# GLAD-RUC/DistEGNN

Hardware: NVIDIA H100
Metric: graph_steps_per_sec (higher is better)
Workload: dtype f32

## Files before the change

### distegnn_b200/csrc/edge_layer_cs.cu

```cuda
#include <cuda_fp16.h>
#include <string.h>

#include "common.cuh"
#include "det.cuh"
#include "tc16.cuh"
#include "tile_mma.cuh"

namespace degnn {

struct EdgeCsArgs {
    int64_t N, E;
    const int32_t* E_dev;
    int A;
    unsigned flags;
    const int32_t* row;
    const int32_t* col;
    const float* ea;
    const float* x4;
    const float* P;
    const float* Q;
    const float* w1r;
    const float* w1e;
    const float* w2;
    const float* b2;
    const float* wc;
    const float* bc;
    const float* w3;
    float* agg_m;
    float* agg_x;
    float* slots;
};

constexpr int CS_WG = 4;
constexpr int CS_THREADS = 128 * CS_WG, CS_WARPS = CS_THREADS / 32;
constexpr int CS_TILE = 64;
constexpr int CS_QROW = 72;
constexpr int CS_WBUF = 16 * CS_QROW;
constexpr int CS_IDX = 64;
constexpr int CS_W = 64 * 64;
constexpr int CS_SMEM_BYTES = 4 * CS_W * 2
                              + CS_WARPS * 2 * 8
                              + (4 * H + DISTEGNN_MAX_EDGE_ATTR * H) * 4
                              + CS_WARPS * 2 * CS_WBUF * 4
                              + CS_WARPS * CS_IDX * 4
                              + CS_WARPS * 16 * 8 * 4;
constexpr uint32_t CS_LBO = 1024;

template <int AT, bool LASTL, bool DET>
__global__ void __launch_bounds__(CS_THREADS, 1) edge_layer_cs_kernel(const EdgeCsArgs a) {
    using namespace tmma;
    constexpr int AMAX = AT >= 0 ? (AT > 0 ? AT : 1) : DISTEGNN_MAX_EDGE_ATTR;
    constexpr int AR = (AT == 1 || AT == 2) ? AT : 0;
    constexpr bool need_m = !LASTL;
    __half* W2hi = reinterpret_cast<__half*>(degnn_dyn_smem);
    __half* W2lo = W2hi + CS_W;
    __half* Wchi = W2lo + CS_W;
    __half* Wclo = Wchi + CS_W;
    uint64_t* bars = reinterpret_cast<uint64_t*>(Wclo + CS_W);
    float* b2s = reinterpret_cast<float*>(bars + CS_WARPS * 2);
    float* bcs = b2s + H;
    float* w3s = bcs + H;
    float* w1rs = w3s + H;
    float* w1es = w1rs + H;
    float* qbufs = w1es + DISTEGNN_MAX_EDGE_ATTR * H;
    int* idx_all = reinterpret_cast<int*>(qbufs + CS_WARPS * 2 * CS_WBUF);
    float* xs_all = reinterpret_cast<float*>(idx_all + CS_WARPS * CS_IDX);

    const int tid = threadIdx.x;
    const int lane = tid & 31;
    const int warp = tid >> 5;
    const int wg = warp >> 2;
    const int w = warp & 3;
    const int g = lane >> 2, q = lane & 3;
    const int A = AT >= 0 ? AT : a.A;
    const bool normalize = a.flags & DISTEGNN_FLAG_NORMALIZE;

    tc16::stage_weight<CS_THREADS>(W2hi, W2lo, a.w2, 0, 64, tid, SILU_T_IN);
    tc16::stage_weight<CS_THREADS>(Wchi, Wclo, a.wc, 0, 64, tid);
    if (tid < H) {
        b2s[tid] = a.b2[tid] * SILU_T_IN;
        bcs[tid] = a.bc[tid] * SILU_T_IN;
        w3s[tid] = a.w3[tid] * SILU_T_OUT;
        w1rs[tid] = a.w1r[tid];
    }
    for (int i = tid; i < DISTEGNN_MAX_EDGE_ATTR * H; i += CS_THREADS) w1es[i] = i < A * H ? a.w1e[i] : 0.f;
    for (int i = tid; i < CS_WARPS * 2 * CS_WBUF / 4; i += CS_THREADS)
        reinterpret_cast<float4*>(qbufs)[i] = make_float4(0.f, 0.f, 0.f, 0.f);
    if (tid == 0) {
        for (int i = 0; i < CS_WARPS * 2; ++i) mbar_init(&bars[i], 1);
        fence_mbar_init();
    }
    fence_proxy_async_smem();
    __syncthreads();

    float* qb = qbufs + warp * 2 * CS_WBUF;
    int* nidx = idx_all + warp * CS_IDX;
    float* xs = xs_all + warp * 16 * 8 + 8 * (lane & 15);
    uint64_t* qbar = bars + 2 * warp;
    const uint64_t bW2hi = make_desc(smem_u32(W2hi), CS_LBO, 128), bW2lo = make_desc(smem_u32(W2lo), CS_LBO, 128);
    const uint64_t bWchi = make_desc(smem_u32(Wchi), CS_LBO, 128), bWclo = make_desc(smem_u32(Wclo), CS_LBO, 128);

    const int64_t nE = a.E_dev ? min((int64_t)__ldg(a.E_dev), a.E) : a.E;
    const int64_t num_tiles = (nE + CS_TILE - 1) / CS_TILE;
    const int64_t stride = (int64_t)gridDim.x * CS_WG;
    int64_t tile = (int64_t)blockIdx.x * CS_WG + wg;

    auto edge_of = [&](int64_t tl) { return tl * CS_TILE + 16 * w + lane; };
    auto has_edge = [&](int64_t tl) { return lane < 16 && tl < num_tiles && edge_of(tl) < nE; };
    auto fetch_q = [&](int64_t tl, int b, int col_e, bool v) {
        if (lane == 0) {
            const int64_t nv = min((int64_t)16, max((int64_t)0, nE - (tl * CS_TILE + 16 * w)));
            mbar_expect_tx(qbar + b, (uint32_t)nv * (H * 4));
        }
        if (v) bulk_g2s(qb + b * CS_WBUF + lane * CS_QROW, a.Q + (size_t)col_e * H, H * 4, qbar + b);
    };

    int row_c = -1;
    float dx = 0.f, dy = 0.f, dz = 0.f, radial = 0.f;
    auto set_geometry = [&](float4 xi, float4 xj) {
        dx = xi.x - xj.x; dy = xi.y - xj.y; dz = xi.z - xj.z;
        radial = dx * dx + dy * dy + dz * dz;
        if (normalize) {
            const float inv = 1.0f / (sqrtf(radial) + 1e-8f);
            dx *= inv; dy *= inv; dz *= inv;
        }
    };
    float ea_c[AR > 0 ? AR : 1], n_ea[AR > 0 ? AR : 1];
#pragma unroll
    for (int k = 0; k < (AR > 0 ? AR : 1); ++k) ea_c[k] = n_ea[k] = 0.f;
    int n_row = -1, n_col = 0;

    if (tile < num_tiles) {
        int col_c = 0;
        if (has_edge(tile)) {
            const int64_t e = edge_of(tile);
            row_c = __ldg(a.row + e);
            col_c = __ldg(a.col + e);
#pragma unroll
            for (int k = 0; k < AR; ++k) ea_c[k] = __ldg(a.ea + e * AR + k);
        }
        fetch_q(tile, 0, col_c, row_c >= 0);
        set_geometry(ldg4(a.x4 + (size_t)max(row_c, 0) * 4), ldg4(a.x4 + (size_t)col_c * 4));
        if (has_edge(tile + stride)) {
            const int64_t e = edge_of(tile + stride);
            n_row = __ldg(a.row + e);
            n_col = __ldg(a.col + e);
#pragma unroll
            for (int k = 0; k < AR; ++k) n_ea[k] = __ldg(a.ea + e * AR + k);
        }
    }

    for (int it = 0; tile < num_tiles; ++it, tile += stride) {
        const int64_t ntile = tile + stride, nntile = ntile + stride;
        const int b = it & 1;
        float* qcur = qb + b * CS_WBUF;

        int cont_row = -1;
        if constexpr (DET) {
            const int64_t e0 = tile * CS_TILE + 16 * w;
            const int r0 = __shfl_sync(FULL, row_c, 0);
            if (r0 >= 0 && e0 > 0 && __ldg(a.row + e0 - 1) == r0) cont_row = r0;
        }
        float* const slot = DET ? a.slots + (size_t)(tile * 4 + w) * DET_EDGE_SLOT : nullptr;

        if (ntile < num_tiles) fetch_q(ntile, b ^ 1, n_col, n_row >= 0);
        if (n_row >= 0) {
            cp_async16(xs, a.x4 + (size_t)n_row * 4);
            cp_async16(xs + 4, a.x4 + (size_t)n_col * 4);
            prefetch_l1(a.P + (size_t)n_row * H);
            prefetch_l1(a.P + (size_t)n_row * H + 32);
        }
        if (has_edge(nntile)) {
            const int64_t e = edge_of(nntile);
            cp_async4(nidx + lane, a.row + e);
            cp_async4(nidx + 16 + lane, a.col + e);
            if (AT == 1) cp_async4(nidx + 32 + 2 * lane, a.ea + e);
            if (AT == 2) cp_async8(nidx + 32 + 2 * lane, a.ea + e * 2);
        }
        cp_async_commit();

        const int ra = __shfl_sync(FULL, row_c, g), rb = __shfl_sync(FULL, row_c, g + 8);
        const float rada = __shfl_sync(FULL, radial, g), radb = __shfl_sync(FULL, radial, g + 8);
        float eaa[AMAX], eab[AMAX];
#pragma unroll
        for (int k = 0; k < AMAX; ++k) {
            if (AR > 0) {
                eaa[k] = __shfl_sync(FULL, ea_c[k < AR ? k : 0], g);
                eab[k] = __shfl_sync(FULL, ea_c[k < AR ? k : 0], g + 8);
            } else if (AT < 0) {
                const int64_t e = tile * CS_TILE + 16 * w + g;
                eaa[k] = (k < A && ra >= 0) ? __ldg(a.ea + e * A + k) : 0.f;
                eab[k] = (k < A && rb >= 0) ? __ldg(a.ea + (e + 8) * A + k) : 0.f;
            } else {
                eaa[k] = eab[k] = 0.f;
            }
        }
        const float* pa = a.P + (size_t)max(ra, 0) * H + 2 * q;
        const float* pb = a.P + (size_t)max(rb, 0) * H + 2 * q;
        const float* qa = qcur + g * CS_QROW + 2 * q;
        const float* qbr = qa + 8 * CS_QROW;
        const bool oka = !DET || ra >= 0, okb = !DET || rb >= 0;
        auto pre = [&](int j, const float* prow, const float* qrow, float rad, const float (&ea)[AMAX], bool ok) {
            if (DET && !ok) return bc2(0.f);
            const int c = 8 * j + 2 * q;
            const f32x2 pp = __ldg(reinterpret_cast<const f32x2*>(prow + 8 * j));
            const f32x2 qq = *reinterpret_cast<const f32x2*>(qrow + 8 * j);
            f32x2 p = fma2(bc2(rad), *reinterpret_cast<const f32x2*>(w1rs + c), add2(pp, qq));
#pragma unroll
            for (int k = 0; k < AMAX; ++k)
                if (AT < 0 || k < A)
                    p = fma2(bc2(ea[k]), *reinterpret_cast<const f32x2*>(w1es + k * H + c), p);
            return p;
        };
        uint32_t ahi[16], alo[16];
        float qmax = 0.f;
        auto silu_guard = [&] { return silu_q_overflow(qmax); };
        tc16::RowScales s1;
        mbar_wait(qbar + b, (uint32_t)((it >> 1) & 1));
        tc16::encode_rows<false, true>(
            [&](int j, f32x2& va, f32x2& vb, auto pass) {
                va = pre(j, pa, qa, rada, eaa, oka);
                vb = pre(j, pb, qbr, radb, eab, okb);
                silu4p<decltype(pass)::value != tc16::FAST_PASS>(va, vb, qmax);
            },
            ahi, alo, s1, silu_guard);

        float d[32];
        tc16::mma_f16x3_rA<CS_LBO>(d, ahi, alo, bW2hi, bW2lo);
        const int row_prev = __shfl_up_sync(FULL, row_c, 1);
        const uint32_t M = __ballot_sync(FULL, lane == 0 || row_prev != row_c) & 0xffffu;
        tc16::mma_f16x3_rA_wait(d, ahi, alo);

        qmax = 0.f;
        tc16::RowScales s2;
        tc16::encode_rows<false>(
            [&](int j, f32x2& ma, f32x2& mb, auto pass) {
                const f32x2 bb = *reinterpret_cast<const f32x2*>(b2s + 8 * j + 2 * q);
                ma = fma2(pk2(d[4 * j + 0], d[4 * j + 1]), bc2(s1.inv_a), bb);
                mb = fma2(pk2(d[4 * j + 2], d[4 * j + 3]), bc2(s1.inv_b), bb);
                silu4t<decltype(pass)::value != tc16::FAST_PASS>(ma, mb, qmax);
                if (need_m && decltype(pass)::value != tc16::ENCODE_PASS) {
                    *reinterpret_cast<f32x2*>(qcur + g * CS_QROW + 8 * j + 2 * q) = ma;
                    *reinterpret_cast<f32x2*>(qcur + (g + 8) * CS_QROW + 8 * j + 2 * q) = mb;
                }
            },
            ahi, alo, s2, silu_guard);

        tc16::mma_f16x3_rA<CS_LBO>(d, ahi, alo, bWchi, bWclo);
        if (need_m) {
            __syncwarp();
            const float* colp = qcur + 2 * lane;
            auto flush = [&](f32x2 acc, int e_last) {
                const int rr = __shfl_sync(FULL, row_c, e_last);
                if (rr >= 0) {
                    float v0, v1;
                    upk2(mul2(acc, bc2(SILU_T_OUT)), v0, v1);
                    if constexpr (DET)
                        *reinterpret_cast<float2*>(rr == cont_row ? slot + 2 * lane : a.agg_m + (size_t)rr * H + 2 * lane) =
                            make_float2(v0, v1);
                    else
                        red_add_v2(a.agg_m + (size_t)rr * H + 2 * lane, v0, v1);
                }
            };
            f32x2 s0 = *reinterpret_cast<const f32x2*>(colp);
            if ((M >> 1) == 0u) {
                f32x2 s1 = *reinterpret_cast<const f32x2*>(colp + CS_QROW);
#pragma unroll
                for (int e = 2; e < 16; e += 2) {
                    s0 = add2(s0, *reinterpret_cast<const f32x2*>(colp + e * CS_QROW));
                    s1 = add2(s1, *reinterpret_cast<const f32x2*>(colp + (e + 1) * CS_QROW));
                }
                flush(add2(s0, s1), 15);
            } else {
#pragma unroll
                for (int e = 1; e < 16; ++e) {
                    const f32x2 v = *reinterpret_cast<const f32x2*>(colp + e * CS_QROW);
                    if ((M >> e) & 1u) {
                        flush(s0, e - 1);
                        s0 = v;
                    } else {
                        s0 = add2(s0, v);
                    }
                }
                flush(s0, 15);
            }
        }
        fence_proxy_async_smem();
        __syncwarp();
        tc16::mma_f16x3_rA_wait(d, ahi, alo);

        float phia, phib;
        tc16::phi_head_t(d, s2.inv_a, s2.inv_b, bcs, w3s, q, phia, phib);
        {
            const float fa = __shfl_sync(FULL, phia, 4 * (lane & 7)), fb = __shfl_sync(FULL, phib, 4 * (lane & 7));
            const float phi = (lane & 8) ? fb : fa;
            float sx = dx * phi, sy = dy * phi, sz = dz * phi;
#pragma unroll
            for (int o = 1; o < 16; o <<= 1) {
                const int rk = __shfl_up_sync(FULL, row_c, o);
                const float ox = __shfl_up_sync(FULL, sx, o), oy = __shfl_up_sync(FULL, sy, o), oz = __shfl_up_sync(FULL, sz, o);
                if (lane >= o && rk == row_c) { sx += ox; sy += oy; sz += oz; }
            }
            const int rnext = __shfl_down_sync(FULL, row_c, 1);
            if (row_c >= 0 && (lane == 15 || rnext != row_c)) {
                if constexpr (DET) {
                    float* dst = row_c == cont_row ? slot + H : a.agg_x + (size_t)row_c * 4;
                    dst[0] = sx;
                    dst[1] = sy;
                    dst[2] = sz;
                } else {
                    float* dst = a.agg_x + (size_t)row_c * 4;
                    atomicAdd(dst + 0, sx);
                    atomicAdd(dst + 1, sy);
                    atomicAdd(dst + 2, sz);
                }
            }
        }

        cp_async_wait_all();
        row_c = n_row;
        float4 xi_n = make_float4(0.f, 0.f, 0.f, 0.f), xj_n = xi_n;
        if (n_row >= 0) {
            xi_n = *reinterpret_cast<const float4*>(xs);
            xj_n = *reinterpret_cast<const float4*>(xs + 4);
        }
        set_geometry(xi_n, xj_n);
#pragma unroll
        for (int k = 0; k < AR; ++k) ea_c[k] = n_ea[k];
        n_row = -1;
        if (has_edge(nntile)) {
            n_row = nidx[lane];
            n_col = nidx[16 + lane];
            if (AT == 1) n_ea[0] = __int_as_float(nidx[32 + 2 * lane]);
            if (AT == 2) {
                n_ea[0] = __int_as_float(nidx[32 + 2 * lane]);
                n_ea[AR - 1] = __int_as_float(nidx[33 + 2 * lane]);
            }
        }
    }
}

}

namespace degnn {

template <bool DET>
static int edge_layer_fwd(int64_t n_nodes, int64_t n_edges, int A, int C, int Na, unsigned flags, const int32_t* row,
                          const int32_t* col, const float* edge_attr_sorted, const float* x4, const float* P,
                          const float* Q, const float* layer_params, float* agg_m, float* agg_x,
                          const int32_t* n_edges_dev, void* workspace, int64_t workspace_bytes, void* stream,
                          int max_ctas) {
    if (int rc = check_dims(A, C, Na)) return rc;
    if (n_edges == 0) return DISTEGNN_OK;
    DEGNN_CHECK_ARG(n_nodes > 0 && n_edges > 0, "negative size");
    DEGNN_CHECK_ARG(row && col && x4 && P && Q && layer_params && agg_x, "null pointer");
    DEGNN_CHECK_ARG(A == 0 || edge_attr_sorted, "null edge_attr with edge_attr_nf > 0");
    DEGNN_CHECK_ARG((flags & DISTEGNN_FLAG_LAST) || agg_m, "null agg_m");
    float* slots = nullptr;
    if (DET) {
        if (int rc = det_check_workspace(n_nodes, n_edges, C, workspace, workspace_bytes, "distegnn_edge_layer_fwd_det"))
            return rc;
        slots = det_edge_slots(workspace, n_nodes, C);
    }
    Layout L = make_layout(A, C, Na);
    EdgeCsArgs a;
    a.N = n_nodes; a.E = n_edges; a.E_dev = n_edges_dev; a.A = A; a.flags = flags & 0xffffu;
    a.row = row; a.col = col; a.ea = edge_attr_sorted; a.x4 = x4; a.P = P; a.Q = Q;
    a.w1r = layer_params + L.off[DISTEGNN_P_E_W1R];
    a.w1e = layer_params + L.off[DISTEGNN_P_E_W1E];
    a.w2 = layer_params + L.off[DISTEGNN_P_E_W2];
    a.b2 = layer_params + L.off[DISTEGNN_P_E_B2];
    a.wc = layer_params + L.off[DISTEGNN_P_E_WC];
    a.bc = layer_params + L.off[DISTEGNN_P_E_BC];
    a.w3 = layer_params + L.off[DISTEGNN_P_E_W3];
    a.agg_m = agg_m; a.agg_x = agg_x; a.slots = slots;
    const int64_t tiles = (n_edges + CS_TILE - 1) / CS_TILE;
    int64_t grid = (tiles + CS_WG - 1) / CS_WG;
    if (grid > sm_count()) grid = sm_count();
    if (DET) grid = det_grid(grid, max_ctas);
    auto launch = [&](auto kern) {
        ensure_dynamic_smem((const void*)kern, (int)CS_SMEM_BYTES);
        kern<<<(unsigned)grid, CS_THREADS, CS_SMEM_BYTES, (cudaStream_t)stream>>>(a);
    };
    const bool last = flags & DISTEGNN_FLAG_LAST;
    switch (A) {
        case 0: last ? launch(edge_layer_cs_kernel<0, true, DET>) : launch(edge_layer_cs_kernel<0, false, DET>); break;
        case 1: last ? launch(edge_layer_cs_kernel<1, true, DET>) : launch(edge_layer_cs_kernel<1, false, DET>); break;
        case 2: last ? launch(edge_layer_cs_kernel<2, true, DET>) : launch(edge_layer_cs_kernel<2, false, DET>); break;
        default: last ? launch(edge_layer_cs_kernel<-1, true, DET>) : launch(edge_layer_cs_kernel<-1, false, DET>); break;
    }
    DEGNN_CHECK_LAUNCH();
    return DISTEGNN_OK;
}

int edge_layer_fwd_det(int64_t n_nodes, int64_t n_edges, int A, int C, int Na, unsigned flags, const int32_t* row,
                       const int32_t* col, const float* edge_attr_sorted, const float* x4, const float* P, const float* Q,
                       const float* layer_params, float* agg_m, float* agg_x, const int32_t* n_edges_dev,
                       void* workspace, int64_t workspace_bytes, void* stream, int max_ctas) {
    return edge_layer_fwd<true>(n_nodes, n_edges, A, C, Na, flags, row, col, edge_attr_sorted, x4, P, Q, layer_params,
                                agg_m, agg_x, n_edges_dev, workspace, workspace_bytes, stream, max_ctas);
}

}

extern "C" int distegnn_edge_layer_fwd(int64_t n_nodes, int64_t n_edges, int A, int C, int Na, unsigned flags,
                                       const int32_t* row, const int32_t* col, const float* edge_attr_sorted,
                                       const float* x4, const float* P, const float* Q,
                                       const float* layer_params, float* agg_m, float* agg_x,
                                       const int32_t* n_edges_dev, void* stream) {
    return degnn::edge_layer_fwd<false>(n_nodes, n_edges, A, C, Na, flags, row, col, edge_attr_sorted, x4, P, Q,
                                        layer_params, agg_m, agg_x, n_edges_dev, nullptr, 0, stream, 0);
}

extern "C" int distegnn_edge_layer_fwd_det(int64_t n_nodes, int64_t n_edges, int A, int C, int Na, unsigned flags,
                                           const int32_t* row, const int32_t* col, const float* edge_attr_sorted,
                                           const float* x4, const float* P, const float* Q,
                                           const float* layer_params, float* agg_m, float* agg_x,
                                           const int32_t* n_edges_dev, void* workspace, int64_t workspace_bytes,
                                           void* stream) {
    return degnn::edge_layer_fwd_det(n_nodes, n_edges, A, C, Na, flags, row, col, edge_attr_sorted, x4, P, Q,
                                     layer_params, agg_m, agg_x, n_edges_dev, workspace, workspace_bytes, stream, 0);
}
```

Before: 34.55.

## Replace TMA bulk Q-row fetch with warp-cooperative cp.async and defer issue

Drops the per-warp mbarriers and TMA bulk_g2s copies of gathered Q rows. Each warp now fetches the rows with 16-byte cp.async, lanes cooperating two rows per step via shuffles, and completion is tracked through the existing cp.async group wait. For fixed attribute counts, issuing the next tile's prefetches is moved to after the first MMA is launched, so they overlap tensor-core work. This removes mbarrier wait and proxy-fence overhead but adds more per-lane instructions and shuffles, and the Q data must now arrive within the same tile iteration.

```diff
diff --git a/distegnn_b200/csrc/edge_layer_cs.cu b/distegnn_b200/csrc/edge_layer_cs.cu
--- a/distegnn_b200/csrc/edge_layer_cs.cu
+++ b/distegnn_b200/csrc/edge_layer_cs.cu
@@ -39,7 +39,6 @@
 constexpr int CS_IDX = 64;
 constexpr int CS_W = 64 * 64;
 constexpr int CS_SMEM_BYTES = 4 * CS_W * 2
-                              + CS_WARPS * 2 * 8
                               + (4 * H + DISTEGNN_MAX_EDGE_ATTR * H) * 4
                               + CS_WARPS * 2 * CS_WBUF * 4
                               + CS_WARPS * CS_IDX * 4
@@ -56,8 +55,7 @@
     __half* W2lo = W2hi + CS_W;
     __half* Wchi = W2lo + CS_W;
     __half* Wclo = Wchi + CS_W;
-    uint64_t* bars = reinterpret_cast<uint64_t*>(Wclo + CS_W);
-    float* b2s = reinterpret_cast<float*>(bars + CS_WARPS * 2);
+    float* b2s = reinterpret_cast<float*>(Wclo + CS_W);
     float* bcs = b2s + H;
     float* w3s = bcs + H;
     float* w1rs = w3s + H;
@@ -86,17 +84,12 @@
     for (int i = tid; i < DISTEGNN_MAX_EDGE_ATTR * H; i += CS_THREADS) w1es[i] = i < A * H ? a.w1e[i] : 0.f;
     for (int i = tid; i < CS_WARPS * 2 * CS_WBUF / 4; i += CS_THREADS)
         reinterpret_cast<float4*>(qbufs)[i] = make_float4(0.f, 0.f, 0.f, 0.f);
-    if (tid == 0) {
-        for (int i = 0; i < CS_WARPS * 2; ++i) mbar_init(&bars[i], 1);
-        fence_mbar_init();
-    }
     fence_proxy_async_smem();
     __syncthreads();
 
     float* qb = qbufs + warp * 2 * CS_WBUF;
     int* nidx = idx_all + warp * CS_IDX;
     float* xs = xs_all + warp * 16 * 8 + 8 * (lane & 15);
-    uint64_t* qbar = bars + 2 * warp;
     const uint64_t bW2hi = make_desc(smem_u32(W2hi), CS_LBO, 128), bW2lo = make_desc(smem_u32(W2lo), CS_LBO, 128);
     const uint64_t bWchi = make_desc(smem_u32(Wchi), CS_LBO, 128), bWclo = make_desc(smem_u32(Wclo), CS_LBO, 128);
 
@@ -107,12 +100,12 @@
 
     auto edge_of = [&](int64_t tl) { return tl * CS_TILE + 16 * w + lane; };
     auto has_edge = [&](int64_t tl) { return lane < 16 && tl < num_tiles && edge_of(tl) < nE; };
-    auto fetch_q = [&](int64_t tl, int b, int col_e, bool v) {
-        if (lane == 0) {
-            const int64_t nv = min((int64_t)16, max((int64_t)0, nE - (tl * CS_TILE + 16 * w)));
-            mbar_expect_tx(qbar + b, (uint32_t)nv * (H * 4));
-        }
-        if (v) bulk_g2s(qb + b * CS_WBUF + lane * CS_QROW, a.Q + (size_t)col_e * H, H * 4, qbar + b);
+    auto fetch_q = [&](int b, int col_v) {
+#pragma unroll
+        for (int i = 0; i < 8; ++i) {
+            const int r = 2 * i + (lane >> 4), c = __shfl_sync(FULL, col_v, r);
+            if (c >= 0) cp_async16(qb + b * CS_WBUF + r * CS_QROW + 4 * (lane & 15), a.Q + (size_t)c * H + 4 * (lane & 15));
+        }
     };
 
     int row_c = -1;
@@ -139,7 +132,8 @@
 #pragma unroll
             for (int k = 0; k < AR; ++k) ea_c[k] = __ldg(a.ea + e * AR + k);
         }
-        fetch_q(tile, 0, col_c, row_c >= 0);
+        fetch_q(0, row_c >= 0 ? col_c : -1);
+        cp_async_commit();
         set_geometry(ldg4(a.x4 + (size_t)max(row_c, 0) * 4), ldg4(a.x4 + (size_t)col_c * 4));
         if (has_edge(tile + stride)) {
             const int64_t e = edge_of(tile + stride);
@@ -148,6 +142,8 @@
 #pragma unroll
             for (int k = 0; k < AR; ++k) n_ea[k] = __ldg(a.ea + e * AR + k);
         }
+        cp_async_wait_all();
+        __syncwarp();
     }
 
     for (int it = 0; tile < num_tiles; ++it, tile += stride) {
@@ -163,21 +159,24 @@
         }
         float* const slot = DET ? a.slots + (size_t)(tile * 4 + w) * DET_EDGE_SLOT : nullptr;
 
-        if (ntile < num_tiles) fetch_q(ntile, b ^ 1, n_col, n_row >= 0);
-        if (n_row >= 0) {
-            cp_async16(xs, a.x4 + (size_t)n_row * 4);
-            cp_async16(xs + 4, a.x4 + (size_t)n_col * 4);
-            prefetch_l1(a.P + (size_t)n_row * H);
-            prefetch_l1(a.P + (size_t)n_row * H + 32);
-        }
-        if (has_edge(nntile)) {
-            const int64_t e = edge_of(nntile);
-            cp_async4(nidx + lane, a.row + e);
-            cp_async4(nidx + 16 + lane, a.col + e);
-            if (AT == 1) cp_async4(nidx + 32 + 2 * lane, a.ea + e);
-            if (AT == 2) cp_async8(nidx + 32 + 2 * lane, a.ea + e * 2);
-        }
-        cp_async_commit();
+        auto requests = [&] {
+            fetch_q(b ^ 1, n_row >= 0 ? n_col : -1);
+            if (n_row >= 0) {
+                cp_async16(xs, a.x4 + (size_t)n_row * 4);
+                cp_async16(xs + 4, a.x4 + (size_t)n_col * 4);
+                prefetch_l1(a.P + (size_t)n_row * H);
+                prefetch_l1(a.P + (size_t)n_row * H + 32);
+            }
+            if (has_edge(nntile)) {
+                const int64_t e = edge_of(nntile);
+                cp_async4(nidx + lane, a.row + e);
+                cp_async4(nidx + 16 + lane, a.col + e);
+                if (AT == 1) cp_async4(nidx + 32 + 2 * lane, a.ea + e);
+                if (AT == 2) cp_async8(nidx + 32 + 2 * lane, a.ea + e * 2);
+            }
+            cp_async_commit();
+        };
+        if constexpr (AT < 0) requests();
 
         const int ra = __shfl_sync(FULL, row_c, g), rb = __shfl_sync(FULL, row_c, g + 8);
         const float rada = __shfl_sync(FULL, radial, g), radb = __shfl_sync(FULL, radial, g + 8);
@@ -216,7 +215,6 @@
         float qmax = 0.f;
         auto silu_guard = [&] { return silu_q_overflow(qmax); };
         tc16::RowScales s1;
-        mbar_wait(qbar + b, (uint32_t)((it >> 1) & 1));
         tc16::encode_rows<false, true>(
             [&](int j, f32x2& va, f32x2& vb, auto pass) {
                 va = pre(j, pa, qa, rada, eaa, oka);
@@ -229,6 +227,7 @@
         tc16::mma_f16x3_rA<CS_LBO>(d, ahi, alo, bW2hi, bW2lo);
         const int row_prev = __shfl_up_sync(FULL, row_c, 1);
         const uint32_t M = __ballot_sync(FULL, lane == 0 || row_prev != row_c) & 0xffffu;
+        if constexpr (AT >= 0) requests();
         tc16::mma_f16x3_rA_wait(d, ahi, alo);
 
         qmax = 0.f;
@@ -285,7 +284,6 @@
                 flush(s0, 15);
             }
         }
-        fence_proxy_async_smem();
         __syncwarp();
         tc16::mma_f16x3_rA_wait(d, ahi, alo);
 
@@ -318,6 +316,7 @@
         }
 
         cp_async_wait_all();
+        __syncwarp();
         row_c = n_row;
         float4 xi_n = make_float4(0.f, 0.f, 0.f, 0.f), xj_n = xi_n;
         if (n_row >= 0) {
```

After: 35.41, median of 6. +2.5%, better.
